# Boese0601/RC-MVSNet

Hardware: AMD Instinct MI355X
Metric: ref-scenes/sec (DTU 3-view 512x640, D=48/32/8) (higher is better)
Workload: dtype f32; 1 GPU; BASELINE configs[1]: CascadeMVSNet_eval.forward, DTU-shaped 3 views 512x640, D=(48,32,8), batch 1 per GPU, fp32, random-init seeded weights; views=3, height=512, width=640, parallelism=scene-per-gpu x1, ranks=1, procs_per_gpu=1, rccl_ranks=0

## Files before the change

### rc_mvsnet_amd/csrc/conv3d.hip

```cpp
#include "common.h"

namespace rcmvs {

enum ConvMode { CONV_S1 = 0, CONV_S2 = 1, CONV_T2 = 2 };

struct ConvDims {
    int B, D, H, W;
    int Do, Ho, Wo;
};

template <int CI, int CO, int MODE>
__global__ __launch_bounds__(256) void conv3d_direct_kernel(
    const float* __restrict__ x, const float* __restrict__ wp, const float* __restrict__ scale,
    const float* __restrict__ shift, const float* __restrict__ res, float* __restrict__ y,
    ConvDims dm, int relu) {
    constexpr int VW = (CI % 4 == 0) ? 4 : 1;
    const long long nvox = (long long)dm.B * dm.Do * dm.Ho * dm.Wo;
    long long t = (long long)blockIdx.x * blockDim.x + threadIdx.x;
    if (t >= nvox) return;
    int ow = (int)(t % dm.Wo);
    long long r = t / dm.Wo;
    int oh = (int)(r % dm.Ho); r /= dm.Ho;
    int od = (int)(r % dm.Do);
    int b = (int)(r / dm.Do);
// ... 79 lines not shown
    if (Ci == CI && Co == CO) {                                                                                   \
        hipLaunchKernelGGL((conv3d_direct_kernel<CI, CO, MODE>), grid, block, 0, st, x, wp, scale, shift, res, y, \
                           dm, relu);                                                                             \
        return launch_status("conv3d_direct");                                                                    \
    }
    RCMVS_CONV_CASE(8, 8) RCMVS_CONV_CASE(16, 8) RCMVS_CONV_CASE(32, 8) RCMVS_CONV_CASE(41, 8) RCMVS_CONV_CASE(44, 8)
    RCMVS_CONV_CASE(8, 16) RCMVS_CONV_CASE(8, 32) RCMVS_CONV_CASE(8, 48) RCMVS_CONV_CASE(16, 16) RCMVS_CONV_CASE(16, 32) RCMVS_CONV_CASE(32, 32)
    RCMVS_CONV_CASE(32, 64) RCMVS_CONV_CASE(64, 64) RCMVS_CONV_CASE(64, 32) RCMVS_CONV_CASE(32, 16)
    RCMVS_CONV_CASE(8, 1)
#undef RCMVS_CONV_CASE
    return fail(-1, "conv3d: unsupported channel pair Ci=%d Co=%d", Ci, Co);
}

int conv3d_mfma_launch(const float* x, const float* wm, const float* scale, const float* shift, const float* res,
                       float* y, int B, int D, int H, int W, int Ci, int Co, int mode, int relu, hipStream_t st, float* ymax = nullptr);
bool conv3d_mfma_supported(int Ci, int Co, int mode);
int pack_weight_mfma_launch(const float* w, float* packed, int Co, int Ci, int transposed, hipStream_t st);
long long mfma_weight_floats_host(int Ci, int Co);

bool conv3d_lds_supported(int Ci, int Co, int stride);
int conv3d_lds_launch(const float* x, const float* wp, const float* scale, const float* shift, const float* res, float* y,
                      int B, int D, int H, int W, int Ci, int Co, int relu, hipStream_t st, int lds_cfg);

bool deconv3d_lds_supported(int Ci, int Co);
int deconv3d_lds_launch(const float* x, const float* wp, const float* scale, const float* shift, const float* res, float* y,
                        int B, int D, int H, int W, int Ci, int Co, int relu, hipStream_t st);

enum { X3_KIND_PLANAR = 3, X3_NKINDS = 4 };
bool conv3d_x3_supported(int Ci, int Co, int kind);
long long conv3d_x3_weight_floats(int Ci, int Co, int kind);
int conv3d_x3_pack(const float* w, float* img, int Co, int Ci, int kind, int transposed, hipStream_t st);
int conv3d_x3_launch(const float* x, const float* wimg, const float* scale, const float* shift, const float* res, float* y,
                     int B, int D, int H, int W, int Ci, int Co, int kind, int relu, hipStream_t st, int max_blocks, int s2d = 0,
                     const float* xmax = nullptr, float* ymax = nullptr);
bool conv3d_x3h_supported(int Ci, int Co, int kind);
long long conv3d_x3h_weight_floats(int Ci, int Co, int kind);
int conv3d_x3h_pack(const float* w, float* img, int Co, int Ci, int kind, int transposed, const float* wsc, hipStream_t st);
int conv3d_x3_wscale(const float* w, int n, float* out, hipStream_t st);

static inline long long direct_weight_floats(int Ci, int Co) { return 27LL * Ci * Co; }
static inline long long x3_image_offset(int Ci, int Co, int kind) {
    long long off = direct_weight_floats(Ci, Co) + (conv3d_mfma_supported(Ci, Co, 0) ? mfma_weight_floats_host(Ci, Co) : 0);
    for (int k = 0; k < kind; ++k) off += conv3d_x3_weight_floats(Ci, Co, k);
    return off;
}
static inline long long x3h_image_offset(int Ci, int Co, int kind) {
    long long off = x3_image_offset(Ci, Co, X3_NKINDS);
    for (int k = 0; k < kind; ++k) off += conv3d_x3h_weight_floats(Ci, Co, k);
    return off;
}
long long prob_pair_weight_floats();
int prob_pair_pack(const float* w, float* img, const float* wsc, hipStream_t st);
static inline bool has_prob_pair(int Ci, int Co) { return Ci == 8 && Co == 1; }
static inline long long prob_pair_image_offset(int Ci, int Co) { return x3h_image_offset(Ci, Co, X3_NKINDS) + 4; }
long long prob_pair_blob_offset() { return prob_pair_image_offset(8, 1); }
bool conv11_prob_supported(int Dt, int Ht, int Wt);
int conv11_prob_launch(const float* t, const float* w11img, const float* scale, const float* shift, const float* res, const float* wprobimg,
                       const float* tmax, const float* rmax, const float* coef, float* y, int B, int Dt, int Ht, int Wt, int zc_force, hipStream_t st,
                       const float* planes, float* depth, float* conf);

}

using namespace rcmvs;

struct ConvImpl {
    bool direct, prefer_lds, no_x3, ysq;
    int lds_cfg, x3_blocks;
    explicit ConvImpl(int on) : direct(on & 1), prefer_lds(!(on & 16)), no_x3((on >> 6) & 1), ysq((on >> 24) & 1),
                                lds_cfg(((on >> 1) & 7) | (((on >> 5) & 1) << 3) | (((on >> 25) & 1) << 4) | (((on >> 16) & 0xff) << 8)), x3_blocks((on >> 8) & 0xff) {}
};

extern "C" {

long long rcmvs_packed_weight_floats(int Co, int Ci) {
    if (Co <= 0 || Ci <= 0) return -1;
    long long n = direct_weight_floats(Ci, Co);
    if (conv3d_mfma_supported(Ci, Co, 0)) n += mfma_weight_floats_host(Ci, Co);
    for (int k = 0; k < X3_NKINDS; ++k) n += conv3d_x3_weight_floats(Ci, Co, k) + conv3d_x3h_weight_floats(Ci, Co, k);
    return n + 4 + (has_prob_pair(Ci, Co) ? prob_pair_weight_floats() : 0);
}

enum ConvSel { SEL_X3_PLANAR, SEL_X3H, SEL_X3, SEL_LDS, SEL_MFMA, SEL_DIRECT };
static ConvSel conv_select(int Ci, int Co, int mode, bool planar, bool scaled, const ConvImpl& im) {
    const bool x3 = !im.direct && !im.no_x3;
    if (mode == CONV_T2) {
        if (scaled && x3 && conv3d_x3h_supported(Ci, Co, CONV_T2)) return SEL_X3H;
        if (x3 && conv3d_x3_supported(Ci, Co, CONV_T2)) return SEL_X3;
        if (deconv3d_lds_supported(Ci, Co) && !im.direct) return SEL_LDS;
        if (conv3d_mfma_supported(Ci, Co, CONV_T2) && !im.direct) return SEL_MFMA;
        return SEL_DIRECT;
    }
    const int stride = mode == CONV_S1 ? 1 : 2;
    if (planar && x3 && conv3d_x3_supported(Ci, Co, X3_KIND_PLANAR)) return SEL_X3_PLANAR;
    if (scaled && x3 && conv3d_x3h_supported(Ci, Co, mode)) return SEL_X3H;
    if (x3 && conv3d_x3_supported(Ci, Co, mode)) return SEL_X3;
    if (im.prefer_lds && conv3d_lds_supported(Ci, Co, stride) && !im.direct) return SEL_LDS;
    if (conv3d_mfma_supported(Ci, Co, mode) && !im.direct) return SEL_MFMA;
    if (conv3d_lds_supported(Ci, Co, stride) && !im.direct) return SEL_LDS;
    return SEL_DIRECT;
}

// ... 34 lines not shown
        if (!(images & (IMG_X3H << k)) || !conv3d_x3h_supported(Ci, Co, k) || ((k == 2) != (transposed == 1))) continue;
        if (!scaled) { rc = conv3d_x3_wscale(w, n, wsc, as_stream(stream)); if (rc) return rc; scaled = true; }
        rc = conv3d_x3h_pack(w, packed + x3h_image_offset(Ci, Co, k), Co, Ci, k, transposed, wsc, as_stream(stream));
        if (rc) return rc;
    }
    if ((images & IMG_PROB_PAIR) && has_prob_pair(Ci, Co) && !transposed) {
        if (!scaled) { rc = conv3d_x3_wscale(w, n, wsc, as_stream(stream)); if (rc) return rc; }
        rc = prob_pair_pack(w, packed + prob_pair_image_offset(Ci, Co), wsc, as_stream(stream));
        if (rc) return rc;
    }
    return 0;
}

int rcmvs_pack_conv3d_weight(const float* w, float* packed, int Co, int Ci, int transposed, void* stream) {
    return rcmvs_pack_conv3d_weight_sel(w, packed, Co, Ci, transposed, IMG_ALL, stream);
}

static int conv3d_dispatch(const float* x, const float* w_packed, const float* scale, const float* shift,
                           const float* residual, float* y,
                           int B, int D, int H, int W, int Ci, int Co, int stride, int relu, void* stream, const ConvImpl& im,
                           const float* xmax = nullptr, float* ymax = nullptr) {
    RCMVS_REQUIRE(x && w_packed && y, "conv3d_fwd: null pointer");
    RCMVS_REQUIRE(B > 0 && D > 0 && H > 0 && W > 0, "conv3d_fwd: bad sizes");
    RCMVS_REQUIRE(stride == 1 || stride == 2, "conv3d_fwd: stride must be 1 or 2");
    RCMVS_REQUIRE((scale == nullptr) == (shift == nullptr), "conv3d_fwd: scale and shift go together");
    ConvDims dm{B, D, H, W, (D - 1) / stride + 1, (H - 1) / stride + 1, (W - 1) / stride + 1};
    hipStream_t st = as_stream(stream);
    const int mode = stride == 1 ? CONV_S1 : CONV_S2;
    const ConvSel sel = conv_select(Ci, Co, mode, stride == 1 && D == 1, xmax != nullptr, im);
    RCMVS_REQUIRE(!im.ysq || (sel == SEL_X3_PLANAR && ymax), "conv3d_scaled_fwd: the squared output bound (impl bit 24) is kept by the planar matrix-core kernels only");
    if (sel == SEL_X3_PLANAR)
        return conv3d_x3_launch(x, w_packed + x3_image_offset(Ci, Co, X3_KIND_PLANAR), scale, shift, residual, y, B, D, H, W, Ci, Co, X3_KIND_PLANAR, relu, st, im.x3_blocks, im.ysq ? 2 : 0, nullptr, ymax);
    if (sel == SEL_X3H)
        return conv3d_x3_launch(x, w_packed + x3h_image_offset(Ci, Co, mode), scale, shift, residual, y, B, D, H, W, Ci, Co, mode, relu, st, im.x3_blocks, 0, xmax, ymax);
    if (sel == SEL_X3)
        return conv3d_x3_launch(x, w_packed + x3_image_offset(Ci, Co, mode), scale, shift, residual, y, B, D, H, W, Ci, Co, mode, relu, st, im.x3_blocks, 0, nullptr, ymax);
    if (sel == SEL_MFMA)
        return conv3d_mfma_launch(x, w_packed + direct_weight_floats(Ci, Co), scale, shift, residual, y, B, D, H, W, Ci, Co,
                                  mode, relu, st, ymax);
    RCMVS_REQUIRE(!ymax, "conv3d_scaled_fwd: no matrix-core kernel for Ci=%d Co=%d stride=%d, the output bound cannot be maintained", Ci, Co, stride);
    if (sel == SEL_LDS)
        return conv3d_lds_launch(x, w_packed, scale, shift, residual, y, B, D, H, W, Ci, Co, relu, st, im.lds_cfg);
    if (stride == 1) return direct_dispatch<CONV_S1>(x, w_packed, scale, shift, residual, y, dm, Ci, Co, relu, st);
    return direct_dispatch<CONV_S2>(x, w_packed, scale, shift, residual, y, dm, Ci, Co, relu, st);
}

int rcmvs_conv3d_fwd(const float* x, const float* w_packed, const float* scale, const float* shift,
                     const float* residual, float* y,
                     int B, int D, int H, int W, int Ci, int Co, int stride, int relu, void* stream) {
    return conv3d_dispatch(x, w_packed, scale, shift, residual, y, B, D, H, W, Ci, Co, stride, relu, stream, ConvImpl(0));
}

int rcmvs_conv3d_scaled_fwd(const float* x, const float* x_absmax, const float* w_packed, const float* scale, const float* shift,
                            const float* residual, float* y, float* y_absmax,
                            int B, int D, int H, int W, int Ci, int Co, int stride, int relu, int impl, void* stream) {
    return conv3d_dispatch(x, w_packed, scale, shift, residual, y, B, D, H, W, Ci, Co, stride, relu, stream, ConvImpl(impl), x_absmax, y_absmax);
}

int rcmvs_conv2d_s2d_fwd(const float* x, const float* w_packed, const float* scale, const float* shift, float* y,
                         int N, int H, int W, int C, int Co, int relu, void* stream) {
    RCMVS_REQUIRE(x && w_packed && y, "conv2d_s2d_fwd: null pointer");
    RCMVS_REQUIRE(N > 0 && H > 0 && W > 0 && H % 2 == 0 && W % 2 == 0, "conv2d_s2d_fwd: H and W must be even (got %d x %d)", H, W);
    RCMVS_REQUIRE((scale == nullptr) == (shift == nullptr), "conv2d_s2d_fwd: scale and shift go together");
    RCMVS_REQUIRE(conv3d_x3_supported(4 * C, Co, X3_KIND_PLANAR), "conv2d_s2d_fwd: no planar split-bf16 kernel for %d -> %d channels", 4 * C, Co);
    return conv3d_x3_launch(x, w_packed + x3_image_offset(4 * C, Co, X3_KIND_PLANAR), scale, shift, nullptr, y, N, 1, H / 2, W / 2, 4 * C, Co,
                            X3_KIND_PLANAR, relu, as_stream(stream), 0, 1);
}
// ... 64 lines not shown
```

### rc_mvsnet_amd/csrc/conv3d_x3.hip

```cpp
#include "common.h"
#include "x3_pieces.h"
#include <atomic>
#include <cstdlib>

#ifndef X3_ABLATION
#define X3_ABLATION 0
#endif

namespace rcmvs {

#if X3_ABLATION
int x3_ablation_mask = 0;
long long* x3_trace_buf = nullptr;
#define X3_STAMP(SLOT) do { if (dm.trace && blockIdx.x == 0 && lane == 0 && s < 64) dm.trace[s * 8 + (SLOT)] = (long long)__builtin_amdgcn_s_memtime(); } while (0)
#else
#define X3_STAMP(SLOT) do { } while (0)
#endif
#define X3_DBG(BIT) (X3_ABLATION == 1 && ((dm.dbg >> (BIT)) & 1))


enum { X3_S1 = 0, X3_S2 = 1, X3_T2 = 2, X3_P1 = 3, X3_KINDS = 4 };
__host__ __device__ constexpr bool x3_unit(int kind) { return kind == X3_S1 || kind == X3_P1; }
enum { X3_XT = 0, X3_YT = 1, X3_PL = 2 };

// ... 640 lines not shown
        if (tid == 0) {
            float m = redmax[0];
#pragma unroll
            for (int i = 1; i < 8; ++i) m = fmaxf(m, redmax[i]);
            if (dm.ysq) m = m * m;
            atomicMax(reinterpret_cast<unsigned int*>(ymax) + (blockIdx.x & 63) * 16, __float_as_uint(m));
        }
    }
}

#define RCMVS_X3_LIST(X) X(8, 8, X3_S1) X(16, 8, X3_S1) X(32, 8, X3_S1) X(16, 16, X3_S1) X(8, 16, X3_S2) X(16, 32, X3_S2) X(16, 8, X3_T2) \
    X(8, 8, X3_P1) X(16, 16, X3_P1) X(32, 32, X3_P1) X(32, 16, X3_P1) X(64, 32, X3_P1) X(32, 32, X3_S1) X(32, 16, X3_T2)
#define RCMVS_X3H_LIST(X) X(8, 8, X3_S1) X(16, 8, X3_S1) X(32, 8, X3_S1) X(16, 16, X3_S1) X(8, 16, X3_S2) X(16, 32, X3_S2) X(16, 8, X3_T2) \
    X(32, 32, X3_S1) X(32, 16, X3_T2)

bool conv3d_x3_supported(int Ci, int Co, int kind) {
#define X3_CASE(CI, CO, K) if (Ci == CI && Co == CO && kind == K) return true;
    RCMVS_X3_LIST(X3_CASE)
#undef X3_CASE
    return false;
}

bool conv3d_deep_supported(int Ci, int Co, int kind);
long long conv3d_deep_weight_floats(int Ci, int Co, int kind);
int conv3d_deep_pack(const float* w, float* img, int Co, int Ci, int kind, int transposed, const float* wsc, hipStream_t st);
int conv3d_deep_launch(const float* x, const float* wimg, const float* scale, const float* shift, const float* res, float* y,
                       int B, int D, int H, int W, int Ci, int Co, int kind, int relu, hipStream_t st, const float* xmax, float* ymax);

bool conv3d_z8_supported(int Ci, int Co, int kind);
bool conv3d_zs2_supported(int Ci, int Co, int kind);
int conv3d_zs2_launch(const float* x, const float* wimg, const float* scale, const float* shift, float* y,
                      int B, int D, int H, int W, int relu, hipStream_t st, int max_blocks, const float* xmax, float* ymax);
int conv3d_z8_launch(const float* x, const float* wimg, const float* scale, const float* shift, float* y,
                     int B, int D, int H, int W, int Ci, int Co, int relu, hipStream_t st, int max_blocks, const float* xmax, float* ymax);

bool conv3d_x3h_supported(int Ci, int Co, int kind) {
    if (conv3d_deep_supported(Ci, Co, kind)) return true;
#define X3_CASE(CI, CO, K) if (Ci == CI && Co == CO && kind == K) return true;
    RCMVS_X3H_LIST(X3_CASE)
#undef X3_CASE
    return false;
}

long long conv3d_x3_weight_floats(int Ci, int Co, int kind) {
#define X3_CASE(CI, CO, K) if (Ci == CI && Co == CO && kind == K) return (long long)X3<CI, CO, K>::KSTEPS * 3 * X3<CI, CO, K>::MT_ALL * 64 * 8 / 2;
    RCMVS_X3_LIST(X3_CASE)
#undef X3_CASE
    return 0;
}

long long conv3d_x3h_weight_floats(int Ci, int Co, int kind) {
    if (conv3d_deep_supported(Ci, Co, kind)) return conv3d_deep_weight_floats(Ci, Co, kind);
#define X3_CASE(CI, CO, K) if (Ci == CI && Co == CO && kind == K) return 4 + (long long)X3<CI, CO, K, 2>::KSTEPS * 2 * X3<CI, CO, K, 2>::MT_ALL * 64 * 8 / 2;
    RCMVS_X3H_LIST(X3_CASE)
#undef X3_CASE
    return 0;
}

int conv3d_x3_pack(const float* w, float* img, int Co, int Ci, int kind, int transposed, hipStream_t st) {
#define X3_CASE(CI, CO, K) if (Ci == CI && Co == CO && kind == K) { \
        const int nthr = X3<CI, CO, K>::KSTEPS * X3<CI, CO, K>::MT_ALL * 64 * 8; \
        hipLaunchKernelGGL((x3_pack_kernel<CI, CO, K, 3>), dim3((nthr + 255) / 256), dim3(256), 0, st, w, reinterpret_cast<unsigned short*>(img), transposed, (const float*)nullptr); \
        return launch_status("conv3d_x3_pack"); }
    RCMVS_X3_LIST(X3_CASE)
#undef X3_CASE
    return fail(-1, "conv3d_x3_pack: unsupported Ci=%d Co=%d kind=%d", Ci, Co, kind);
}
// ... 46 lines not shown
            dm.stepcap = (int)((spb + 2 + 3) & ~3LL);
            const size_t ldsb = (size_t)C::LDSB + (size_t)dm.itemcap * 16 + (size_t)dm.stepcap * 4 + 64;
            if (ldsb <= 160 * 1024) {
                const int grid_b = (int)(T < n_blk ? T : n_blk);
                static std::atomic<bool> attr_set_b[64];
                if (!attr_set_b[dev].load(std::memory_order_acquire)) { (void)hipFuncSetAttribute((const void*)conv3d_x3_kernel<CI, CO, K, NP>, hipFuncAttributeMaxDynamicSharedMemorySize, 160 * 1024); attr_set_b[dev].store(true, std::memory_order_release); }
                hipLaunchKernelGGL((conv3d_x3_kernel<CI, CO, K, NP>), dim3((unsigned)grid_b), dim3(512), ldsb, st, x, reinterpret_cast<const x3_u32x4*>(wimg), scale, shift, res, y, dm, xmax, ymax);
                return launch_status("conv3d_x3");
            }
            dm.bal = 0;
        }
    }
    int grid_n = dm.nitems < n_blk ? dm.nitems : n_blk;
    size_t lds = 0;
    for (;;) {
        const long long per_blk = (items + grid_n - 1) / grid_n + 2;
        dm.itemcap = (int)((per_blk + 3) & ~3LL);
        dm.stepcap = (int)(((long long)dm.itemcap * dm.zchunk + 3) & ~3LL);
        lds = (size_t)C::LDSB + (size_t)dm.itemcap * 16 + (size_t)dm.stepcap * 4 + 64;
        if (lds <= 160 * 1024 || grid_n >= dm.nitems) break;
        grid_n = grid_n * 2 < dm.nitems ? grid_n * 2 : dm.nitems;
    }
    if (lds > 160 * 1024) return fail(-1, "conv3d_x3: the schedule of a block does not fit the LDS (%zu bytes)", lds);
    if (dm.zchunk >= 32768 || dm.itemcap >= 32768) return fail(-1, "conv3d_x3: schedule descriptor fields overflow");
    dim3 grid((unsigned)grid_n);
    static std::atomic<bool> attr_set[64];
    if (!attr_set[dev].load(std::memory_order_acquire)) { (void)hipFuncSetAttribute((const void*)conv3d_x3_kernel<CI, CO, K, NP>, hipFuncAttributeMaxDynamicSharedMemorySize, 160 * 1024); attr_set[dev].store(true, std::memory_order_release); }
    hipLaunchKernelGGL((conv3d_x3_kernel<CI, CO, K, NP>), grid, dim3(512), lds, st, x, reinterpret_cast<const x3_u32x4*>(wimg), scale, shift, res, y, dm, xmax, ymax);
    return launch_status("conv3d_x3");
}

int conv3d_x3_launch(const float* x, const float* wimg, const float* scale, const float* shift, const float* res, float* y,
                     int B, int D, int H, int W, int Ci, int Co, int kind, int relu, hipStream_t st, int max_blocks, int s2d,
                     const float* xmax, float* ymax) {
    if (xmax && conv3d_deep_supported(Ci, Co, kind)) return conv3d_deep_launch(x, wimg, scale, shift, res, y, B, D, H, W, Ci, Co, kind, relu, st, xmax, ymax);
    if (xmax && !res && !s2d && conv3d_z8_supported(Ci, Co, kind)) {
        const int rc = conv3d_z8_launch(x, wimg, scale, shift, y, B, D, H, W, Ci, Co, relu, st, max_blocks, xmax, ymax);
        if (rc != 1) return rc;
    }
    if (xmax && !res && !s2d && conv3d_zs2_supported(Ci, Co, kind)) {
        const int rc = conv3d_zs2_launch(x, wimg, scale, shift, y, B, D, H, W, relu, st, max_blocks, xmax, ymax);
        if (rc != 1) return rc;
    }
    const int ysq = (s2d >> 1) & 1;
    s2d &= 1;
    if (s2d && (kind != X3_P1 || Ci % 16 != 0)) return fail(-1, "conv3d_x3: the space-to-depth view needs the planar kind and Ci a multiple of 16");
    if ((long long)B * D * H * W * Ci * 4 >= 0x7ffffff0LL) return fail(-1, "conv3d_x3: input tensor too large for 32-bit offsets");
    {
        const long long so = kind == X3_T2 ? 8 : (kind == X3_S2 ? 1 : 1);
        if ((long long)B * D * H * W * so * Co * 4 >= 0x7ffffff0LL) return fail(-1, "conv3d_x3: output tensor too large for 32-bit offsets");
    }
    constexpr int MAXDEV = 64;
    static std::atomic<int> cu_of[MAXDEV];
    int dev = 0;
    if (hipGetDevice(&dev) != hipSuccess || dev < 0 || dev >= MAXDEV) return fail(-1, "conv3d_x3: cannot query the device");
    if (cu_of[dev] == 0) {
        hipDeviceProp_t prop;
        if (hipGetDeviceProperties(&prop, dev) != hipSuccess) return fail(-1, "conv3d_x3: cannot query the device");
        cu_of[dev] = prop.multiProcessorCount > 0 ? prop.multiProcessorCount : 256;
    }
    const int n_cu = cu_of[dev];
    const int n_blk = max_blocks > 0 ? max_blocks : n_cu;
    X3Dims dm;
    dm.B = B; dm.D = D; dm.H = H; dm.W = W; dm.relu = relu; dm.s2d = s2d; dm.ysq = ysq; dm.dbg = 0; dm.trace = nullptr;
    dm.place = 0;
#if X3_ABLATION
    dm.dbg = x3_ablation_mask;
    dm.trace = x3_trace_buf;
#endif
    if (kind == X3_T2) { dm.Do = 2 * D; dm.Ho = 2 * H; dm.Wo = 2 * W; }
// ... 18 lines not shown
```

### rc_mvsnet_amd/csrc/conv3d_z8.hip

```cpp
#include "common.h"
#include "x3_pieces.h"
#include <atomic>
#include <cstdlib>

namespace rcmvs {

template <int CIN, int COUT>
struct Z8 {
    static constexpr bool XT = COUT == 8 && CIN == 8, YT = COUT == 8 && CIN >= 16, PL = COUT == 16;
    static constexpr bool ALO = CIN == 32;
#ifndef Z8_PL_NTW
#define Z8_PL_NTW 1
#endif
    static constexpr int NTW = YT ? 1 : (PL ? Z8_PL_NTW : 2);
    static constexpr int NTT = 8 * NTW;
    static constexpr int TY = PL ? NTT / 2 : NTT, TX = 32;
    static constexpr int RSTEP = PL ? 4 : 8;
    static constexpr int VB = CIN * 2;
    static constexpr int Q4 = CIN / 4;
    static constexpr int PPS = 32 / CIN;
    static constexpr int QR = YT ? 4 : 3, QC = XT ? 4 : 3, PPKD = QR * QC;
    static constexpr int SPK = (PPKD + PPS - 1) / PPS;
    static constexpr int KSTEPS = 3 * SPK;
    static constexpr int TYP = TY + 2, TXP = TX + 2;
    static constexpr int ROWB = TXP * VB, PLB = TYP * ROWB, SLB = 2 * PLB;
    static constexpr int NSLOT = 2;
    static constexpr int NLD = (TYP * TXP * Q4 + 511) / 512;
    static constexpr int CS = XT ? 2 : 1;
    static constexpr int ALOB = ALO ? KSTEPS * 1024 : 0;
    static constexpr int LDS = NSLOT * SLB + ALOB + 64;
    static_assert((COUT == 8 && (CIN == 8 || CIN == 16 || CIN == 32)) || (COUT == 16 && CIN == 16), "conv0 of stages 3, 2 and 1, conv2");
    static_assert(LDS <= 160 * 1024, "LDS budget");
};

template <int CIN> __device__ __forceinline__ int z8_swz(int hc) { return CIN == 32 ? ((hc >> 2) & 1) * 32 : 0; }

struct Z8Dims {
    int B, D, H, W;
    int tiles_x, ntiles;
    int relu;
};

struct Z8Plan { int nticks, L0, a00, tile0, zb0, nz0, last, nz_last, D; unsigned inv; };
__device__ __forceinline__ bool z8_entry(const Z8Plan& p, int s, int& tile, int& ip, int& zb, int& nz) {
    if (s >= p.nticks) return false;
    if (s < p.L0) { tile = p.tile0; ip = s + p.a00; zb = p.zb0; nz = p.nz0; return true; }
    const int x = s - p.L0;
    const int k1 = p.D == 1 ? x : (int)__umulhi((unsigned)x, p.inv);
    tile = p.tile0 + 1 + k1; ip = x - k1 * p.D + 1; zb = 0;
    nz = (1 + k1 == p.last) ? p.nz_last : p.D;
    return true;
}

template <int CIN, int COUT>
__global__ __launch_bounds__(512) void conv3d_z8_kernel(
    const float* __restrict__ x, const x3_u32x4* __restrict__ wimg, const float* __restrict__ scale, const float* __restrict__ shift,
    float* __restrict__ y, Z8Dims dm, const float* __restrict__ xmax, float* __restrict__ ymax) {
    using C = Z8<CIN, COUT>;
    constexpr int KSTEPS = C::KSTEPS, NLD = C::NLD, OOB = 0x7ffffff0;
    extern __shared__ __attribute__((aligned(16))) x3_byte smem[];
    x3_byte* const alo = smem + C::NSLOT * C::SLB;
    float* const redmax = reinterpret_cast<float*>(alo + C::ALOB);
    const int tid = threadIdx.x, lane = tid & 63;
    const int wave = __builtin_amdgcn_readfirstlane(tid >> 6);
    const int n = lane & 15, kk = lane >> 4;
    const int nblk = gridDim.x, bid = blockIdx.x;
    const int r = ((nblk & 7) == 0) ? (bid & 7) * (nblk >> 3) + (bid >> 3) : bid;
    const long long T = (long long)dm.B * dm.ntiles * dm.D;
    const long long lo = T * r / nblk, hi = T * (r + 1) / nblk;
    if (hi <= lo) return;
    Z8Plan pl;
    {
        const int S = (int)(hi - lo);
        pl.tile0 = (int)(lo / dm.D); pl.zb0 = (int)(lo % dm.D);
        pl.nz0 = min(dm.D - pl.zb0, S);
        const int R = S - pl.nz0, full = R / dm.D, tail = R % dm.D;
        const int nitems = 1 + full + (tail > 0);
        pl.last = nitems - 1; pl.nz_last = tail > 0 ? tail : dm.D;
        pl.a00 = pl.zb0 == 0 ? 1 : 0;
        pl.L0 = pl.nz0 + 2 - pl.a00 - (pl.zb0 + pl.nz0 == dm.D ? 1 : 0); pl.D = dm.D;
        pl.inv = (unsigned)(0x100000000ull / (unsigned)dm.D) + 1u;
        pl.nticks = pl.L0 + full * dm.D + (tail > 0 ? tail + 1 : 0);
    }

    float bound = xmax[lane * 16];
#pragma unroll
    for (int m = 32; m > 0; m >>= 1) bound = fmaxf(bound, __shfl_xor(bound, m));
    float xinv;
    const float xs_scale = x3_pow2_scale(bound, xinv);
    const float unscale = xinv * reinterpret_cast<const float*>(wimg)[1];
    x3_u32x4 wr[KSTEPS][C::ALO ? 1 : 2];
    int boff[C::SPK];
    const int toff = C::XT ? wave * C::ROWB : (wave >> 1) * (C::YT ? 2 : 1) * C::ROWB + (wave & 1) * 16 * C::VB;
#pragma unroll
    for (int j = 0; j < KSTEPS; ++j) {
#pragma unroll
        for (int p = 0; p < (C::ALO ? 1 : 2); ++p) wr[j][p] = wimg[1 + (j * 2 + p) * 64 + lane];
        if (C::ALO && wave == (j & 7)) *reinterpret_cast<x3_u32x4*>(alo + (j * 64 + lane) * 16) = wimg[1 + (j * 2 + 1) * 64 + lane];
    }
#pragma unroll
    for (int js = 0; js < C::SPK; ++js) {
        int q = js * C::PPS + kk / (4 / C::PPS);
        const int ci0 = (kk % (4 / C::PPS)) * 8;
        if (q >= C::PPKD) q = 0;
        const int hc = q % C::QC + n * C::CS;
        boff[js] = toff + (q / C::QC) * C::ROWB + hc * C::VB + ((ci0 * 2) ^ z8_swz<CIN>(hc));
    }
    const int co0 = C::PL ? kk * 4 : (kk & 1) * 4;
    const x3_f32x4 sc = (scale ? *reinterpret_cast<const x3_f32x4*>(scale + co0) : (x3_f32x4){1.f, 1.f, 1.f, 1.f}) * unscale;
    const x3_f32x4 sh = shift ? *reinterpret_cast<const x3_f32x4*>(shift + co0) : (x3_f32x4){0.f, 0.f, 0.f, 0.f};
    const int oyl = C::XT ? wave : (C::YT ? 2 * (wave >> 1) + (kk >> 1) : (wave >> 1)), oxl = C::XT ? 2 * n + (kk >> 1) : (wave & 1) * 16 + n;

    int loff[NLD], hyx[NLD];
#pragma unroll
    for (int i = 0; i < NLD; ++i) {
        static_assert(NLD * 512 - C::TYP * C::TXP * C::Q4 <= 512 && C::TYP * C::TXP * C::Q4 >= 512, "the repeated share exists");
        const int e0 = tid + i * 512, e = e0 >= C::TYP * C::TXP * C::Q4 ? e0 - 512 : e0, v = e / C::Q4, c4 = e % C::Q4;
        const int hy = v / C::TXP, hx = v % C::TXP;
        loff[i] = hy * C::ROWB + hx * C::VB + ((c4 * 8) ^ z8_swz<CIN>(hx));
        hyx[i] = (hy << 20) | (hx << 8) | c4;
    }
    __amdgpu_buffer_rsrc_t rsrc = __builtin_amdgcn_make_buffer_rsrc(const_cast<float*>(x), (short)0, (int)((long long)dm.B * dm.D * dm.H * dm.W * CIN * 4), 0x00020000);
    const int zstride = dm.H * dm.W * CIN * 4;
    __amdgpu_buffer_rsrc_t yrs = __builtin_amdgcn_make_buffer_rsrc(y, (short)0, (int)((long long)dm.B * dm.D * dm.H * dm.W * COUT * 4), 0x00020000);

    int goff[NLD];
    int f_tile = -1;
    auto fetch = [&](x3_f32x4 (&q)[NLD], int sf) {
        int tile, ip, zb, nz;
        const bool valid = z8_entry(pl, sf, tile, ip, zb, nz);
        bool zin = false;
        int zoff = 0;
        if (valid) {
            if (tile != f_tile) {
                f_tile = tile;
                const int b = tile / dm.ntiles, t = tile % dm.ntiles;
                const int y0 = (t / dm.tiles_x) * C::TY, x0 = (t % dm.tiles_x) * C::TX;
                const int base = (((b * dm.D) * dm.H + (y0 - 1)) * dm.W + (x0 - 1)) * CIN * 4;
#pragma unroll
                for (int i = 0; i < NLD; ++i) {
                    const int hy = hyx[i] >> 20, hx = (hyx[i] >> 8) & 0xfff, c4 = hyx[i] & 0xff;
                    const int gy = y0 - 1 + hy, gx = x0 - 1 + hx;
                    goff[i] = (gy >= 0 && gy < dm.H && gx >= 0 && gx < dm.W) ? base + ((hy * dm.W + hx) * CIN + c4 * 4) * 4 : OOB;
                }
            }
            const int z = zb - 1 + ip;
            zin = z >= 0 && z < dm.D;
            zoff = zin ? z * zstride : 0;
        }
#pragma unroll
        for (int i = 0; i < NLD; ++i) q[i] = __builtin_bit_cast(x3_f32x4, __builtin_amdgcn_raw_buffer_load_b128(rsrc, zin ? goff[i] : OOB, zoff, 0));
    };
    auto stash = [&](const x3_f32x4 (&q)[NLD], int slot) {
        x3_byte* sb = smem + slot * C::SLB;
#pragma unroll
        for (int i = 0; i < NLD; ++i) {
            x3_u32x2 h, l;
            x3_split4h(q[i] * xs_scale, h, l);
            *reinterpret_cast<x3_u32x2*>(sb + loff[i]) = h;
            *reinterpret_cast<x3_u32x2*>(sb + C::PLB + loff[i]) = l;
        }
    };

    int ob[C::NTW];
#pragma unroll
    for (int i = 0; i < C::NTW; ++i) ob[i] = OOB;
    const int ostep = dm.H * dm.W * COUT * 4;
    float vmax = 0.0f;
    constexpr int QD = C::ALO ? 1 : 2;
    x3_f32x4 pq[QD][NLD];
    fetch(pq[0], 0);
    if constexpr (QD == 2) fetch(pq[1], 1);
    stash(pq[0], 0);
    fetch(pq[0], QD);
    __syncthreads();
    x3_f32x4 acc[C::NTW][3];
    auto tick = [&](int t, x3_f32x4 (&q)[NLD]) {
        stash(q, (t + 1) & 1);
        fetch(q, t + 1 + QD);
        int ctile, ip, czb, cnz;
        z8_entry(pl, t, ctile, ip, czb, cnz);
        {
            if (ip == (czb == 0 ? 1 : 0)) {
#pragma unroll
                for (int i = 0; i < C::NTW; ++i)
#pragma unroll
                    for (int c = 0; c < 3; ++c) acc[i][c] = (x3_f32x4){0.f, 0.f, 0.f, 0.f};
                const int b = ctile / dm.ntiles, tl = ctile % dm.ntiles;
#pragma unroll
                for (int i = 0; i < C::NTW; ++i) {
                    const int oy = (tl / dm.tiles_x) * C::TY + oyl + C::RSTEP * i, ox = (tl % dm.tiles_x) * C::TX + oxl;
                    ob[i] = (oy < dm.H && ox < dm.W) ? (((((b * dm.D) + czb) * dm.H + oy) * dm.W + ox) * COUT + co0) * 4 : OOB;
                }
            }
            const x3_byte* sb = smem + (t & 1) * C::SLB;
            constexpr int NBQ = C::ALO ? 1 : 2;
            x3_u32x4 bq[NBQ][C::NTW][2];
            auto read_b = [&](int buf, int js) {
#pragma unroll
                for (int i = 0; i < C::NTW; ++i) {
                    const x3_byte* pb = sb + boff[js] + i * C::RSTEP * C::ROWB;
                    bq[buf][i][0] = *reinterpret_cast<const x3_u32x4*>(pb);
                    bq[buf][i][1] = *reinterpret_cast<const x3_u32x4*>(pb + C::PLB);
                }
            };
            if (NBQ == 2) read_b(0, 0);
#pragma unroll
            for (int js = 0; js < C::SPK; ++js) {
                if (NBQ == 1) read_b(0, js);
                else if (js + 1 < C::SPK) read_b((js + 1) & 1, js + 1);
                __builtin_amdgcn_sched_barrier(0);
#pragma unroll
                for (int p = 0; p < 3; ++p) {
#pragma unroll
                    for (int kd = 0; kd < 3; ++kd) {
                        const int j = kd * C::SPK + js;
                        x3_u32x4 a;
                        if constexpr (C::ALO) a = p == 2 ? *reinterpret_cast<const x3_u32x4*>(alo + (j * 64 + lane) * 16) : wr[j][0];
                        else a = wr[j][p == 2 ? 1 : 0];
#pragma unroll
                        for (int i = 0; i < C::NTW; ++i)
                            acc[i][kd] = x3_mfma<2>(a, bq[js & (NBQ - 1)][i][p == 1 ? 1 : 0], acc[i][kd]);
                    }
                }
                __builtin_amdgcn_sched_barrier(0);
            }
            if (ip >= 2) {
#pragma unroll
                for (int i = 0; i < C::NTW; ++i) {
                    x3_f32x4 v = acc[i][2] * sc + sh;
                    if (dm.relu) v = __builtin_elementwise_max(v, (x3_f32x4){0.f, 0.f, 0.f, 0.f});
                    __builtin_amdgcn_raw_buffer_store_b128(__builtin_bit_cast(x3_u32x4, v), yrs, ob[i], 0, 0);
                    const bool in = ob[i] != OOB;
                    vmax = in ? x3_absmax4(vmax, v) : vmax;
                    ob[i] = in ? ob[i] + ostep : OOB;
                }
            }
            if (ip == cnz && czb + cnz == dm.D) {
#pragma unroll
                for (int i = 0; i < C::NTW; ++i) {
                    x3_f32x4 v = acc[i][1] * sc + sh;
                    if (dm.relu) v = __builtin_elementwise_max(v, (x3_f32x4){0.f, 0.f, 0.f, 0.f});
                    __builtin_amdgcn_raw_buffer_store_b128(__builtin_bit_cast(x3_u32x4, v), yrs, ob[i], 0, 0);
                    vmax = ob[i] != OOB ? x3_absmax4(vmax, v) : vmax;
                }
            }
#pragma unroll
            for (int i = 0; i < C::NTW; ++i) { acc[i][2] = acc[i][1]; acc[i][1] = acc[i][0]; acc[i][0] = (x3_f32x4){0.f, 0.f, 0.f, 0.f}; }
        }
        __syncthreads();
    };
    for (int t = 0; t < pl.nticks; t += 2) {
        tick(t, pq[QD - 1]);
        if (t + 1 < pl.nticks) tick(t + 1, pq[0]);
    }
    if (ymax) {
#pragma unroll
        for (int m = 32; m > 0; m >>= 1) vmax = fmaxf(vmax, __shfl_xor(vmax, m));
        if (lane == 0) redmax[wave] = vmax;
        __syncthreads();
        if (tid == 0) {
            float m = redmax[0];
#pragma unroll
            for (int i = 1; i < 8; ++i) m = fmaxf(m, redmax[i]);
            atomicMax(reinterpret_cast<unsigned int*>(ymax) + (blockIdx.x & 63) * 16, __float_as_uint(m));
        }
    }
}

bool conv3d_z8_supported(int Ci, int Co, int kind) {
    static const bool conv2 = [] { const char* e = getenv("RCMVS_Z8_CONV2"); return !e || e[0] != '0'; }();
    return kind == 0 && ((Co == 8 && (Ci == 8 || Ci == 16 || Ci == 32)) || (conv2 && Ci == 16 && Co == 16));
}

template <int CIN, int COUT>
static int z8_launch_t(const float* x, const float* wimg, const float* scale, const float* shift, float* y, const Z8Dims& dm, int n_cu, int dev,
                       const float* xmax, float* ymax, hipStream_t st) {
    using C = Z8<CIN, COUT>;
    constexpr int MAXDEV = 64;
    static std::atomic<bool> raised[MAXDEV];
    if (C::LDS > 64 * 1024 && !raised[dev].load(std::memory_order_acquire)) {
        if (hipFuncSetAttribute((const void*)conv3d_z8_kernel<CIN, COUT>, hipFuncAttributeMaxDynamicSharedMemorySize, C::LDS) != hipSuccess)
            return fail(-1, "conv3d_z8: cannot raise the dynamic LDS limit to %d bytes", C::LDS);
        raised[dev].store(true, std::memory_order_release);
    }
    const long long T = (long long)dm.B * dm.ntiles * dm.D;
    const int blocks = (int)(T < n_cu ? T : n_cu);
    hipLaunchKernelGGL((conv3d_z8_kernel<CIN, COUT>), dim3(blocks), dim3(512), C::LDS, st, x, reinterpret_cast<const x3_u32x4*>(wimg), scale, shift, y, dm, xmax, ymax);
    return launch_status("conv3d_z8");
}

int conv3d_z8_launch(const float* x, const float* wimg, const float* scale, const float* shift, float* y,
                     int B, int D, int H, int W, int Ci, int Co, int relu, hipStream_t st, int max_blocks, const float* xmax, float* ymax) {
    if (!xmax) return fail(-1, "conv3d_z8: the fp16-pair form needs a bound of max|x|");
    if ((long long)B * D * H * W * (Ci > Co ? Ci : Co) * 4 >= 0x7ffffff0LL) return fail(-1, "conv3d_z8: tensor too large for 32-bit offsets");
    constexpr int MAXDEV = 64;
    static std::atomic<int> cu_of[MAXDEV];
    int dev = 0;
    if (hipGetDevice(&dev) != hipSuccess || dev < 0 || dev >= MAXDEV) return fail(-1, "conv3d_z8: cannot query the device");
    if (cu_of[dev] == 0) {
        hipDeviceProp_t prop;
        if (hipGetDeviceProperties(&prop, dev) != hipSuccess) return fail(-1, "conv3d_z8: cannot query the device");
        cu_of[dev] = prop.multiProcessorCount > 0 ? prop.multiProcessorCount : 256;
    }
    Z8Dims dm;
    dm.B = B; dm.D = D; dm.H = H; dm.W = W; dm.relu = relu;
    const int ty = Co == 16 ? Z8<16, 16>::TY : (Ci == 8 ? Z8<8, 8>::TY : Z8<16, 8>::TY);
    dm.tiles_x = (W + 31) / 32;
    dm.ntiles = dm.tiles_x * ((H + ty - 1) / ty);
    const int n_blk = max_blocks > 0 ? max_blocks : cu_of[dev].load();
    if (((long long)B * dm.ntiles * D + n_blk - 1) / n_blk + 2 >= 65536)
        return 1;
    if (Ci == 8 && Co == 8) return z8_launch_t<8, 8>(x, wimg, scale, shift, y, dm, n_blk, dev, xmax, ymax, st);
    if (Ci == 16 && Co == 8) return z8_launch_t<16, 8>(x, wimg, scale, shift, y, dm, n_blk, dev, xmax, ymax, st);
    if (Ci == 32 && Co == 8) return z8_launch_t<32, 8>(x, wimg, scale, shift, y, dm, n_blk, dev, xmax, ymax, st);
    if (Ci == 16 && Co == 16) return z8_launch_t<16, 16>(x, wimg, scale, shift, y, dm, n_blk, dev, xmax, ymax, st);
    return fail(-1, "conv3d_z8: unsupported Ci=%d Co=%d", Ci, Co);
}

}
```

Before: 1004 ref-scenes/s.

## Hold Ci=32 z8 conv weights in AGPRs with 4-wave blocks instead of LDS

Adds an AGPR variant of the fp16-pair z8 3D convolution for Ci=32, Co=8. Blocks shrink to 256 threads, each wave computes two output rows over two 16-column halves, and the high weight steps are fed to inline-asm MFMA from accumulator registers instead of being staged in LDS. This becomes the default path, with a new impl bit to fall back to the LDS-weight form. It drops the LDS weight traffic and its footprint, at the cost of hand-placed s_nop fences, inline asm and fewer waves per block, which may lower latency hiding.

Result: no change. 1010 ref-scenes/s (median of 6 runs) (+0.6%).

```diff
diff --git a/rc_mvsnet_amd/csrc/conv3d.hip b/rc_mvsnet_amd/csrc/conv3d.hip
--- a/rc_mvsnet_amd/csrc/conv3d.hip
+++ b/rc_mvsnet_amd/csrc/conv3d.hip
@@ -135,7 +135,7 @@
 int conv3d_x3_pack(const float* w, float* img, int Co, int Ci, int kind, int transposed, hipStream_t st);
 int conv3d_x3_launch(const float* x, const float* wimg, const float* scale, const float* shift, const float* res, float* y,
                      int B, int D, int H, int W, int Ci, int Co, int kind, int relu, hipStream_t st, int max_blocks, int s2d = 0,
-                     const float* xmax = nullptr, float* ymax = nullptr);
+                     const float* xmax = nullptr, float* ymax = nullptr, int z8_lds_weights = 0);
 bool conv3d_x3h_supported(int Ci, int Co, int kind);
 long long conv3d_x3h_weight_floats(int Ci, int Co, int kind);
 int conv3d_x3h_pack(const float* w, float* img, int Co, int Ci, int kind, int transposed, const float* wsc, hipStream_t st);
@@ -167,9 +167,9 @@
 using namespace rcmvs;
 
 struct ConvImpl {
-    bool direct, prefer_lds, no_x3, ysq;
+    bool direct, prefer_lds, no_x3, ysq, z8_lds;
     int lds_cfg, x3_blocks;
-    explicit ConvImpl(int on) : direct(on & 1), prefer_lds(!(on & 16)), no_x3((on >> 6) & 1), ysq((on >> 24) & 1),
+    explicit ConvImpl(int on) : direct(on & 1), prefer_lds(!(on & 16)), no_x3((on >> 6) & 1), ysq((on >> 24) & 1), z8_lds((on >> 26) & 1),
                                 lds_cfg(((on >> 1) & 7) | (((on >> 5) & 1) << 3) | (((on >> 25) & 1) << 4) | (((on >> 16) & 0xff) << 8)), x3_blocks((on >> 8) & 0xff) {}
 };
 
@@ -270,7 +270,7 @@
     if (sel == SEL_X3_PLANAR)
         return conv3d_x3_launch(x, w_packed + x3_image_offset(Ci, Co, X3_KIND_PLANAR), scale, shift, residual, y, B, D, H, W, Ci, Co, X3_KIND_PLANAR, relu, st, im.x3_blocks, im.ysq ? 2 : 0, nullptr, ymax);
     if (sel == SEL_X3H)
-        return conv3d_x3_launch(x, w_packed + x3h_image_offset(Ci, Co, mode), scale, shift, residual, y, B, D, H, W, Ci, Co, mode, relu, st, im.x3_blocks, 0, xmax, ymax);
+        return conv3d_x3_launch(x, w_packed + x3h_image_offset(Ci, Co, mode), scale, shift, residual, y, B, D, H, W, Ci, Co, mode, relu, st, im.x3_blocks, 0, xmax, ymax, im.z8_lds);
     if (sel == SEL_X3)
         return conv3d_x3_launch(x, w_packed + x3_image_offset(Ci, Co, mode), scale, shift, residual, y, B, D, H, W, Ci, Co, mode, relu, st, im.x3_blocks, 0, nullptr, ymax);
     if (sel == SEL_MFMA)
diff --git a/rc_mvsnet_amd/csrc/conv3d_x3.hip b/rc_mvsnet_amd/csrc/conv3d_x3.hip
--- a/rc_mvsnet_amd/csrc/conv3d_x3.hip
+++ b/rc_mvsnet_amd/csrc/conv3d_x3.hip
@@ -696,7 +696,7 @@
 int conv3d_zs2_launch(const float* x, const float* wimg, const float* scale, const float* shift, float* y,
                       int B, int D, int H, int W, int relu, hipStream_t st, int max_blocks, const float* xmax, float* ymax);
 int conv3d_z8_launch(const float* x, const float* wimg, const float* scale, const float* shift, float* y,
-                     int B, int D, int H, int W, int Ci, int Co, int relu, hipStream_t st, int max_blocks, const float* xmax, float* ymax);
+                     int B, int D, int H, int W, int Ci, int Co, int relu, hipStream_t st, int max_blocks, const float* xmax, float* ymax, int lds_weights);
 
 bool conv3d_x3h_supported(int Ci, int Co, int kind) {
     if (conv3d_deep_supported(Ci, Co, kind)) return true;
@@ -809,10 +809,10 @@
 
 int conv3d_x3_launch(const float* x, const float* wimg, const float* scale, const float* shift, const float* res, float* y,
                      int B, int D, int H, int W, int Ci, int Co, int kind, int relu, hipStream_t st, int max_blocks, int s2d,
-                     const float* xmax, float* ymax) {
+                     const float* xmax, float* ymax, int z8_lds_weights) {
     if (xmax && conv3d_deep_supported(Ci, Co, kind)) return conv3d_deep_launch(x, wimg, scale, shift, res, y, B, D, H, W, Ci, Co, kind, relu, st, xmax, ymax);
     if (xmax && !res && !s2d && conv3d_z8_supported(Ci, Co, kind)) {
-        const int rc = conv3d_z8_launch(x, wimg, scale, shift, y, B, D, H, W, Ci, Co, relu, st, max_blocks, xmax, ymax);
+        const int rc = conv3d_z8_launch(x, wimg, scale, shift, y, B, D, H, W, Ci, Co, relu, st, max_blocks, xmax, ymax, z8_lds_weights);
         if (rc != 1) return rc;
     }
     if (xmax && !res && !s2d && conv3d_zs2_supported(Ci, Co, kind)) {
diff --git a/rc_mvsnet_amd/csrc/conv3d_z8.hip b/rc_mvsnet_amd/csrc/conv3d_z8.hip
--- a/rc_mvsnet_amd/csrc/conv3d_z8.hip
+++ b/rc_mvsnet_amd/csrc/conv3d_z8.hip
@@ -5,17 +5,21 @@
 
 namespace rcmvs {
 
-template <int CIN, int COUT>
+template <int CIN, int COUT, bool AGF = false>
 struct Z8 {
     static constexpr bool XT = COUT == 8 && CIN == 8, YT = COUT == 8 && CIN >= 16, PL = COUT == 16;
-    static constexpr bool ALO = CIN == 32;
+    static constexpr bool AG = AGF;
+    static constexpr bool ALO = CIN == 32 && !AG;
+    static constexpr int NW = AG ? 4 : 8, NT = NW * 64;
+    static_assert(!AG || (CIN == 32 && COUT == 8), "the AGPR form is conv0 of stage 1");
+    static constexpr int VHI = 12, QD = AG || ALO ? 1 : 2;
 #ifndef Z8_PL_NTW
 #define Z8_PL_NTW 1
 #endif
-    static constexpr int NTW = YT ? 1 : (PL ? Z8_PL_NTW : 2);
-    static constexpr int NTT = 8 * NTW;
+    static constexpr int NTW = AG ? 2 : YT ? 1 : (PL ? Z8_PL_NTW : 2);
+    static constexpr int NTT = NW * NTW;
     static constexpr int TY = PL ? NTT / 2 : NTT, TX = 32;
-    static constexpr int RSTEP = PL ? 4 : 8;
+    static constexpr int RSTEP = AG ? 0 : (PL ? 4 : 8), CSTEP = AG ? 16 : 0;
     static constexpr int VB = CIN * 2;
     static constexpr int Q4 = CIN / 4;
     static constexpr int PPS = 32 / CIN;
@@ -25,7 +29,7 @@
     static constexpr int TYP = TY + 2, TXP = TX + 2;
     static constexpr int ROWB = TXP * VB, PLB = TYP * ROWB, SLB = 2 * PLB;
     static constexpr int NSLOT = 2;
-    static constexpr int NLD = (TYP * TXP * Q4 + 511) / 512;
+    static constexpr int NLD = (TYP * TXP * Q4 + NT - 1) / NT;
     static constexpr int CS = XT ? 2 : 1;
     static constexpr int ALOB = ALO ? KSTEPS * 1024 : 0;
     static constexpr int LDS = NSLOT * SLB + ALOB + 64;
@@ -52,12 +56,30 @@
     return true;
 }
 
-template <int CIN, int COUT>
-__global__ __launch_bounds__(512) void conv3d_z8_kernel(
+__device__ __forceinline__ x3_f32x4 z8_mfma(bool asm_form, bool agpr, x3_u32x4 a, x3_u32x4 b, x3_f32x4 c) {
+#if defined(__AMDGCN__)
+    if (asm_form) {
+        if (agpr) asm volatile("v_mfma_f32_16x16x32_f16 %0, %1, %2, %0" : "+v"(c) : "a"(a), "v"(b));
+        else asm volatile("v_mfma_f32_16x16x32_f16 %0, %1, %2, %0" : "+v"(c) : "v"(a), "v"(b));
+        return c;
+    }
+#endif
+    return x3_mfma<2>(a, b, c);
+}
+__device__ __forceinline__ void z8_mfma_fence() {
+    __builtin_amdgcn_sched_barrier(0);
+#if defined(__AMDGCN__)
+    asm volatile("s_nop 15" ::: "memory");
+#endif
+    __builtin_amdgcn_sched_barrier(0);
+}
+
+template <int CIN, int COUT, bool AGF>
+__global__ __launch_bounds__((Z8<CIN, COUT, AGF>::NT)) void conv3d_z8_kernel(
     const float* __restrict__ x, const x3_u32x4* __restrict__ wimg, const float* __restrict__ scale, const float* __restrict__ shift,
     float* __restrict__ y, Z8Dims dm, const float* __restrict__ xmax, float* __restrict__ ymax) {
-    using C = Z8<CIN, COUT>;
-    constexpr int KSTEPS = C::KSTEPS, NLD = C::NLD, OOB = 0x7ffffff0;
+    using C = Z8<CIN, COUT, AGF>;
+    constexpr int KSTEPS = C::KSTEPS, NLD = C::NLD, NT = C::NT, OOB = 0x7ffffff0;
     extern __shared__ __attribute__((aligned(16))) x3_byte smem[];
     x3_byte* const alo = smem + C::NSLOT * C::SLB;
     float* const redmax = reinterpret_cast<float*>(alo + C::ALOB);
@@ -91,7 +113,7 @@
     const float unscale = xinv * reinterpret_cast<const float*>(wimg)[1];
     x3_u32x4 wr[KSTEPS][C::ALO ? 1 : 2];
     int boff[C::SPK];
-    const int toff = C::XT ? wave * C::ROWB : (wave >> 1) * (C::YT ? 2 : 1) * C::ROWB + (wave & 1) * 16 * C::VB;
+    const int toff = C::AG ? wave * 2 * C::ROWB : C::XT ? wave * C::ROWB : (wave >> 1) * (C::YT ? 2 : 1) * C::ROWB + (wave & 1) * 16 * C::VB;
 #pragma unroll
     for (int j = 0; j < KSTEPS; ++j) {
 #pragma unroll
@@ -109,13 +131,14 @@
     const int co0 = C::PL ? kk * 4 : (kk & 1) * 4;
     const x3_f32x4 sc = (scale ? *reinterpret_cast<const x3_f32x4*>(scale + co0) : (x3_f32x4){1.f, 1.f, 1.f, 1.f}) * unscale;
     const x3_f32x4 sh = shift ? *reinterpret_cast<const x3_f32x4*>(shift + co0) : (x3_f32x4){0.f, 0.f, 0.f, 0.f};
-    const int oyl = C::XT ? wave : (C::YT ? 2 * (wave >> 1) + (kk >> 1) : (wave >> 1)), oxl = C::XT ? 2 * n + (kk >> 1) : (wave & 1) * 16 + n;
+    const int oyl = C::AG ? 2 * wave + (kk >> 1) : C::XT ? wave : (C::YT ? 2 * (wave >> 1) + (kk >> 1) : (wave >> 1));
+    const int oxl = C::AG ? n : C::XT ? 2 * n + (kk >> 1) : (wave & 1) * 16 + n;
 
     int loff[NLD], hyx[NLD];
 #pragma unroll
     for (int i = 0; i < NLD; ++i) {
-        static_assert(NLD * 512 - C::TYP * C::TXP * C::Q4 <= 512 && C::TYP * C::TXP * C::Q4 >= 512, "the repeated share exists");
-        const int e0 = tid + i * 512, e = e0 >= C::TYP * C::TXP * C::Q4 ? e0 - 512 : e0, v = e / C::Q4, c4 = e % C::Q4;
+        static_assert(NLD * NT - C::TYP * C::TXP * C::Q4 <= NT && C::TYP * C::TXP * C::Q4 >= NT, "the repeated share exists");
+        const int e0 = tid + i * NT, e = e0 >= C::TYP * C::TXP * C::Q4 ? e0 - NT : e0, v = e / C::Q4, c4 = e % C::Q4;
         const int hy = v / C::TXP, hx = v % C::TXP;
         loff[i] = hy * C::ROWB + hx * C::VB + ((c4 * 8) ^ z8_swz<CIN>(hx));
         hyx[i] = (hy << 20) | (hx << 8) | c4;
@@ -167,7 +190,7 @@
     for (int i = 0; i < C::NTW; ++i) ob[i] = OOB;
     const int ostep = dm.H * dm.W * COUT * 4;
     float vmax = 0.0f;
-    constexpr int QD = C::ALO ? 1 : 2;
+    constexpr int QD = C::QD;
     x3_f32x4 pq[QD][NLD];
     fetch(pq[0], 0);
     if constexpr (QD == 2) fetch(pq[1], 1);
@@ -189,7 +212,7 @@
                 const int b = ctile / dm.ntiles, tl = ctile % dm.ntiles;
 #pragma unroll
                 for (int i = 0; i < C::NTW; ++i) {
-                    const int oy = (tl / dm.tiles_x) * C::TY + oyl + C::RSTEP * i, ox = (tl % dm.tiles_x) * C::TX + oxl;
+                    const int oy = (tl / dm.tiles_x) * C::TY + oyl + C::RSTEP * i, ox = (tl % dm.tiles_x) * C::TX + oxl + C::CSTEP * i;
                     ob[i] = (oy < dm.H && ox < dm.W) ? (((((b * dm.D) + czb) * dm.H + oy) * dm.W + ox) * COUT + co0) * 4 : OOB;
                 }
             }
@@ -199,12 +222,13 @@
             auto read_b = [&](int buf, int js) {
 #pragma unroll
                 for (int i = 0; i < C::NTW; ++i) {
-                    const x3_byte* pb = sb + boff[js] + i * C::RSTEP * C::ROWB;
+                    const x3_byte* pb = sb + boff[js] + i * (C::RSTEP * C::ROWB + C::CSTEP * C::VB);
                     bq[buf][i][0] = *reinterpret_cast<const x3_u32x4*>(pb);
                     bq[buf][i][1] = *reinterpret_cast<const x3_u32x4*>(pb + C::PLB);
                 }
             };
             if (NBQ == 2) read_b(0, 0);
+            if constexpr (C::AG) z8_mfma_fence();
 #pragma unroll
             for (int js = 0; js < C::SPK; ++js) {
                 if (NBQ == 1) read_b(0, js);
@@ -220,11 +244,12 @@
                         else a = wr[j][p == 2 ? 1 : 0];
 #pragma unroll
                         for (int i = 0; i < C::NTW; ++i)
-                            acc[i][kd] = x3_mfma<2>(a, bq[js & (NBQ - 1)][i][p == 1 ? 1 : 0], acc[i][kd]);
+                            acc[i][kd] = z8_mfma(C::AG, p == 2 || j >= C::VHI, a, bq[js & (NBQ - 1)][i][p == 1 ? 1 : 0], acc[i][kd]);
                     }
                 }
                 __builtin_amdgcn_sched_barrier(0);
             }
+            if constexpr (C::AG) z8_mfma_fence();
             if (ip >= 2) {
 #pragma unroll
                 for (int i = 0; i < C::NTW; ++i) {
@@ -247,6 +272,14 @@
             }
 #pragma unroll
             for (int i = 0; i < C::NTW; ++i) { acc[i][2] = acc[i][1]; acc[i][1] = acc[i][0]; acc[i][0] = (x3_f32x4){0.f, 0.f, 0.f, 0.f}; }
+#if defined(__AMDGCN__)
+            if constexpr (C::AG) {
+#pragma unroll
+                for (int i = 0; i < C::NTW; ++i)
+#pragma unroll
+                    for (int c = 0; c < 3; ++c) asm volatile("" : "+v"(acc[i][c]));
+            }
+#endif
         }
         __syncthreads();
     };
@@ -262,7 +295,7 @@
         if (tid == 0) {
             float m = redmax[0];
 #pragma unroll
-            for (int i = 1; i < 8; ++i) m = fmaxf(m, redmax[i]);
+            for (int i = 1; i < C::NW; ++i) m = fmaxf(m, redmax[i]);
             atomicMax(reinterpret_cast<unsigned int*>(ymax) + (blockIdx.x & 63) * 16, __float_as_uint(m));
         }
     }
@@ -273,25 +306,25 @@
     return kind == 0 && ((Co == 8 && (Ci == 8 || Ci == 16 || Ci == 32)) || (conv2 && Ci == 16 && Co == 16));
 }
 
-template <int CIN, int COUT>
+template <int CIN, int COUT, bool AGF = false>
 static int z8_launch_t(const float* x, const float* wimg, const float* scale, const float* shift, float* y, const Z8Dims& dm, int n_cu, int dev,
                        const float* xmax, float* ymax, hipStream_t st) {
-    using C = Z8<CIN, COUT>;
+    using C = Z8<CIN, COUT, AGF>;
     constexpr int MAXDEV = 64;
     static std::atomic<bool> raised[MAXDEV];
     if (C::LDS > 64 * 1024 && !raised[dev].load(std::memory_order_acquire)) {
-        if (hipFuncSetAttribute((const void*)conv3d_z8_kernel<CIN, COUT>, hipFuncAttributeMaxDynamicSharedMemorySize, C::LDS) != hipSuccess)
+        if (hipFuncSetAttribute((const void*)conv3d_z8_kernel<CIN, COUT, AGF>, hipFuncAttributeMaxDynamicSharedMemorySize, C::LDS) != hipSuccess)
             return fail(-1, "conv3d_z8: cannot raise the dynamic LDS limit to %d bytes", C::LDS);
         raised[dev].store(true, std::memory_order_release);
     }
     const long long T = (long long)dm.B * dm.ntiles * dm.D;
     const int blocks = (int)(T < n_cu ? T : n_cu);
-    hipLaunchKernelGGL((conv3d_z8_kernel<CIN, COUT>), dim3(blocks), dim3(512), C::LDS, st, x, reinterpret_cast<const x3_u32x4*>(wimg), scale, shift, y, dm, xmax, ymax);
+    hipLaunchKernelGGL((conv3d_z8_kernel<CIN, COUT, AGF>), dim3(blocks), dim3(C::NT), C::LDS, st, x, reinterpret_cast<const x3_u32x4*>(wimg), scale, shift, y, dm, xmax, ymax);
     return launch_status("conv3d_z8");
 }
 
 int conv3d_z8_launch(const float* x, const float* wimg, const float* scale, const float* shift, float* y,
-                     int B, int D, int H, int W, int Ci, int Co, int relu, hipStream_t st, int max_blocks, const float* xmax, float* ymax) {
+                     int B, int D, int H, int W, int Ci, int Co, int relu, hipStream_t st, int max_blocks, const float* xmax, float* ymax, int lds_weights) {
     if (!xmax) return fail(-1, "conv3d_z8: the fp16-pair form needs a bound of max|x|");
     if ((long long)B * D * H * W * (Ci > Co ? Ci : Co) * 4 >= 0x7ffffff0LL) return fail(-1, "conv3d_z8: tensor too large for 32-bit offsets");
     constexpr int MAXDEV = 64;
@@ -313,6 +346,7 @@
         return 1;
     if (Ci == 8 && Co == 8) return z8_launch_t<8, 8>(x, wimg, scale, shift, y, dm, n_blk, dev, xmax, ymax, st);
     if (Ci == 16 && Co == 8) return z8_launch_t<16, 8>(x, wimg, scale, shift, y, dm, n_blk, dev, xmax, ymax, st);
+    if (Ci == 32 && Co == 8 && !lds_weights) return z8_launch_t<32, 8, true>(x, wimg, scale, shift, y, dm, n_blk, dev, xmax, ymax, st);
     if (Ci == 32 && Co == 8) return z8_launch_t<32, 8>(x, wimg, scale, shift, y, dm, n_blk, dev, xmax, ymax, st);
     if (Ci == 16 && Co == 16) return z8_launch_t<16, 16>(x, wimg, scale, shift, y, dm, n_blk, dev, xmax, ymax, st);
     return fail(-1, "conv3d_z8: unsupported Ci=%d Co=%d", Ci, Co);
```
